# cbg-ethz/BnpC

Hardware: AMD Instinct MI355X
Metric: MCMC steps/s, 5k cells x 1k muts (+ cell x cluster log-lik evals/s in ll_evals_per_s_K0) (higher is better)
Workload: dtype f64

## Files before the change

### bnpc_amd/_lib.py

```python
import ctypes as C
import os
import re

import numpy as np

_PKG = os.path.dirname(os.path.abspath(__file__))
LIB_PATH = os.environ.get('BNPC_LIB') or os.path.join(_PKG, 'libbnpc_hip.so')

_environ_raw = getattr(os.environ, '_data', None)
if not isinstance(_environ_raw, dict) \
        or (_environ_raw and not isinstance(next(iter(_environ_raw)), bytes)):
    _environ_raw = None


def env(name, default=None):
    if _environ_raw is None:
        return os.environ.get(name, default)
    val = _environ_raw.get(name.encode() if isinstance(name, str) else name)
    return default if val is None else os.fsdecode(val)


MAX_VIEWS = 7
TILE_SLOTS = 4
MAX_TRIALS = 4
# ... 149 lines not shown
    'bnpc_view_set_slot': (C.c_int, [_ctx, C.c_int, _pi64, _i64, C.c_int]),
    'bnpc_view_size': (C.c_int, [_ctx, C.c_int, _pi64]),
    'bnpc_ll_theta': (C.c_int, [_ctx, C.c_int, _pf, _i64, C.c_double,
        C.c_double, _pd, _i64]),
    'bnpc_ll_theta_pinned': (C.c_int, [_ctx, C.c_int, _pf, _i64, C.c_double,
        C.c_double, _i64, _ppd]),
    'bnpc_ll_theta_pinned_top2': (C.c_int, [_ctx, C.c_int, _pf, _i64,
        C.c_double, C.c_double, _i64, _pd, _ppd, C.POINTER(C.c_void_p)]),
    'bnpc_ll_theta_pinned_top2_issue': (C.c_int, [_ctx, C.c_int, _pf, _i64,
        C.c_double, C.c_double, _i64, _pd, _ppd, C.POINTER(C.c_void_p)]),
    'bnpc_matrix_wait': (C.c_int, [_ctx]),
    'bnpc_hints_wait': (C.c_int, [_ctx]),
    'bnpc_ll_theta_pinned_sums_issue': (C.c_int, [_ctx, C.c_int, _pf, _i64,
        C.c_double, C.c_double, _i64, _pd, _ppd]),
    'bnpc_hints_in_order_issue': (C.c_int, [_ctx, _pi64,
        C.POINTER(C.c_void_p)]),
    'bnpc_theta_put': (C.c_int, [_ctx, _i64, _pf, _i64]),
    'bnpc_ll_rows_pinned': (C.c_int, [_ctx, C.c_int, _pi64, _i64, C.c_double,
        C.c_double, _i64, _ppd]),
    'bnpc_ll_rows_issue': (C.c_int, [_ctx, C.c_int, _pi64, _i64, C.c_double,
        C.c_double, _i64, C.c_int]),
    'bnpc_ll_rows_wait': (C.c_int, [_ctx, C.c_int, _ppd]),
    'bnpc_ll_rows_issue_hint': (C.c_int, [_ctx, C.c_int, _pi64, _i64,
        C.c_double, C.c_double, _i64, C.c_int, _pd]),
    'bnpc_ll_rows_wait_hint': (C.c_int, [_ctx, C.c_int, _ppd,
        C.POINTER(C.c_void_p)]),
    'bnpc_ll_tables': (C.c_int, [_ctx, C.c_int, _pd, _pd, _i64, _pd, _i64]),
    'bnpc_colcounts': (C.c_int, [_ctx, _pi64, _pi64, _i64, _pi32, _pi32]),
    'bnpc_view_counts': (C.c_int, [_ctx, C.c_int, _pi64, _i64, _pi32, _pi32]),
    'bnpc_colcounts_by_label': (C.c_int, [_ctx, _pi64, _pi64, _i64, _pi32,
# ... 71 lines not shown
        C.POINTER(C.c_void_p), C.POINTER(_i64)]),
    'bnpc_post_fetch': (C.c_int, [C.c_void_p, _pi32, _pd]),
    'bnpc_post_mpear': (C.c_int, [C.c_void_p, C.c_void_p, _i64, _pi64]),
    'bnpc_post_genotypes': (C.c_int, [C.c_void_p, _pi32, _i64, _pf, _i64,
        _i64, _i64, _pd]),
    'bnpc_post_ward': (C.c_int, [C.c_void_p, _pd]),
    'bnpc_post_ward_stats': (C.c_int, [C.c_void_p, C.POINTER(_i64),
        C.POINTER(_i64)]),
    'bnpc_post_destroy': (C.c_int, [C.c_void_p]),
    'bnpc_rg_scan': (C.c_int, [C.POINTER(MT19937), C.c_int, _i64, _pd,
        C.c_double, _pi64, _pi64, _pd]),
    'bnpc_mt_gamma': (C.c_int, [C.POINTER(MT19937), C.c_void_p, C.c_double,
        C.c_double, C.POINTER(C.c_double)]),
    'bnpc_chain_open': (C.c_int, [C.POINTER(ChainState)]),
    'bnpc_chain_close': (C.c_int, [C.POINTER(ChainState)]),
    'bnpc_chain_step': (C.c_int, [_ctx, C.c_void_p, C.POINTER(MT19937),
        C.POINTER(ChainState)]),
    'bnpc_chain_update_alpha': (C.c_int, [C.c_void_p, C.POINTER(MT19937),
        C.POINTER(ChainState)]),
    'bnpc_gamma_logpdf_scalar': (C.c_int, [C.c_void_p, C.c_double, C.c_double,
        C.c_double, C.POINTER(C.c_double), C.POINTER(C.c_int)]),
}

_lib = None


def load():
    global _lib
    if _lib is not None:
        return _lib
# ... 857 lines not shown
    return None if status.value else out.value


class NativeChain:

    def __init__(self, N, M):
        self.st = ChainState()
        self.st.N, self.st.M = N, M
        self.ids = np.zeros(N, dtype=np.int64)
        self.sizes = np.zeros(N, dtype=np.int64)
        self.st.ids, self.st.sizes = ptr(self.ids), ptr(self.sizes)
        self.keep = []
        self._lib = load()
        check(self._lib.bnpc_chain_open(C.byref(self.st)), 'chain_open')

    def close(self):
        if getattr(self, 'st', None) is not None and self.st.work:
            self._lib.bnpc_chain_close(C.byref(self.st))

    def __del__(self):
        try:
            self.close()
        except Exception:
            pass


def tn_ppf_scalar(kernels, q, a, b, loc, scale):
    out, status = C.c_double(0.0), C.c_int(0)
    check(load().bnpc_tn_ppf_scalar(C.addressof(kernels), q, a, b, loc, scale,
        C.byref(out), C.byref(status)), 'tn_ppf_scalar')
# ... 184 lines not shown
        check(self._lib.bnpc_hints_in_order_issue(self._h,
            ptr(order, C.c_int64), C.byref(hint)), 'hints_in_order_issue')
        if not hint.value or n == 0:
            return None
        raw = (C.c_char * (n * TOP2.itemsize)).from_address(hint.value)
        return np.frombuffer(raw, dtype=TOP2, count=n)

    def ll_theta_pinned_top2_in_order(self, view, theta, FP, FN, ld,
                col_prior, order):
        mat = self.ll_theta_pinned_sums_issue(view, theta, FP, FN, ld,
            col_prior)
        hint = self.hints_in_order_issue(order)
        self.hints_wait()
        return mat, hint

    def hints_wait(self):
        check(self._lib.bnpc_hints_wait(self._h), 'hints_wait')

    def matrix_wait(self):
        check(self._lib.bnpc_matrix_wait(self._h), 'matrix_wait')

    def matrix_wait_hook(self):
        return (C.cast(self._lib.bnpc_matrix_wait, C.c_void_p).value,
            self._h.value if hasattr(self._h, 'value') else self._h)

    def theta_put(self, row0, theta):
        theta = np.ascontiguousarray(theta, dtype=np.float32)
        if theta.ndim == 1:
            theta = theta[None, :]
        assert theta.shape[1] == self.M
# ... 198 lines not shown
```

### bnpc_amd/csrc/bnpc_ctx.h

```cpp
#ifndef BNPC_CTX_H
#define BNPC_CTX_H
#include <hip/hip_runtime.h>
#include <stdint.h>
#include <string.h>
#include <algorithm>
#include <vector>

#include "bnpc_hip.h"
#include "bnpc_internal.h"

#define HIPCHK(expr)                                                         \
    do {                                                                     \
        hipError_t e_ = (expr);                                              \
        if (e_ != hipSuccess) {                                              \
            bnpc_set_error("%s failed: %s (%s:%d)", #expr,                   \
                           hipGetErrorString(e_), __FILE__, __LINE__);       \
            return 1;                                                        \
        }                                                                    \
    } while (0)

#define ARGCHK(cond, msg)                                                    \
    do {                                                                     \
        if (!(cond)) {                                                       \
            bnpc_set_error("bad argument: %s", msg);                         \
// ... 85 lines not shown
    char *zc_out_dev = nullptr;
    void *hint_pin = nullptr;
    size_t hint_cap = 0;
    DevBuf hint_prior;
    void *hint_prior_pin = nullptr;
    struct {
        int state = 0;
        int64_t n = 0, K = 0, ldo = 0;
        size_t bytes = 0;
        Top2Prior prior;
        void *hint_dev = nullptr;
        double *rows_dev = nullptr;
    } hint_later;
    void *order_pin = nullptr;
    DevBuf order_dev;
    void *mh_pin = nullptr;
    char *mh_dev = nullptr;
    size_t mh_cap = 0;
    size_t mh_capE = 0;
    struct MhAhead *ahead = nullptr;
    int64_t ahead_begun = 0, ahead_taken = 0, ahead_rows_taken = 0;
    double mh_flagged_share = 0.25;
    hipEvent_t mh_ev[2] = {};
    int64_t screened = 0, screen_kept = 0;
    size_t pin_lazy_bytes = 0;
    bool matrix_eager = false, lazy_fetched = false, pin_copy_queued = false;
    hipEvent_t ev_hints = nullptr;
    unsigned *done_count = nullptr;
    unsigned *done_pin = nullptr;
    unsigned *done_dev = nullptr;
// ... 161 lines not shown
```

### bnpc_amd/csrc/bnpc_internal.h

```cpp
#ifndef BNPC_INTERNAL_H
#define BNPC_INTERNAL_H
#include <math.h>
#include <stdarg.h>
#include <stdint.h>

#include "bnpc_hip.h"

void bnpc_set_error(const char *fmt, ...);

#ifdef __cplusplus
#include <linux/futex.h>
#include <stdlib.h>
#include <sys/syscall.h>
#include <time.h>
#include <unistd.h>

#include <atomic>
#include <functional>
#include <thread>

static inline void bnpc_cpu_relax()
{
#if defined(__x86_64__)
    __builtin_ia32_pause();
// ... 69 lines not shown
                            int64_t *col_of_id, int64_t *col_id,
                            int64_t *col_size, int64_t *order);
double bnpc_legacy_gamma(bnpc_mt19937 *rng, bnpc_legacy_gauss *g, double shape,
                         double scale);

void bnpc_mh_rank0_hook(const std::function<void()> *hook);
void bnpc_mh_row_gate(const std::function<bool(int64_t)> *gate);
#ifdef __cplusplus
int bnpc_mh_ahead_begin(bnpc_ctx *c, const bnpc_mt19937 *rng,
                        const bnpc_legacy_gauss *g,
                        const std::function<bool(bnpc_mt19937 *,
                                                 bnpc_legacy_gauss *)> &prelude,
                        int64_t rows, int64_t M, int64_t n_sd, bool *posted,
                        int64_t min_entries = -1);
void bnpc_mh_ahead_drop(bnpc_ctx *c);
void bnpc_mh_ahead_scan(bnpc_ctx *c, const bnpc_mt19937 *rng, int64_t uniforms,
                        int64_t rows, int64_t M, int64_t n_sd);
void bnpc_rg_scan_order_hook(const std::function<void()> *hook);
void bnpc_move_last_draw_hook(const std::function<void(int)> *hook);
#endif
int bnpc_ll_theta_begin(bnpc_ctx *c, int view, const float *theta, int64_t K,
                        double FP, double FN, double *out, int64_t ldo);
int bnpc_ll_theta_end(bnpc_ctx *c);
int bnpc_rg_scan_step_with(bnpc_ctx *ctx, const bnpc_host_kernels *k,
                           bnpc_mt19937 *rng, int view, int64_t n,
                           int64_t *rg_assignment, double DP_a,
                           const bnpc_mh_args *mh, int32_t *n1, int32_t *n0,
                           double *scan_log_prob, int *status,
                           const double *ll_ready);
int bnpc_rg_counts_and_batch(bnpc_ctx *c, const bnpc_host_kernels *k,
// ... 141 lines not shown
```

### bnpc_amd/csrc/bnpc_kernels.hip

```cpp

#include <hip/hip_runtime.h>
#include <hip/hip_ext.h>
#include <stdint.h>
#include <stdio.h>
#include <stdlib.h>
#include <string.h>
#include <math.h>
#include <vector>
#include <algorithm>

#include "bnpc_ctx.h"

struct LaunchTimers {
    bool on = false;
    std::vector<hipEvent_t> ev;
    size_t used = 0;
    hipEvent_t *next_pair()
    {
        if (used + 2 > ev.size()) {
            const size_t old = ev.size();
            ev.resize(old + 512, nullptr);
            for (size_t i = old; i < ev.size(); i++)
                if (hipEventCreate(&ev[i]) != hipSuccess) {
                    ev.resize(i & ~(size_t)1);
// ... 677 lines not shown
    const double2 *__restrict__ src, double2 *__restrict__ dst, long long n2)
{
    const long long i = (long long)blockIdx.x * 256 + threadIdx.x;
    if (i < n2) dst[i] = src[i];
}

__device__ __forceinline__ void top2_floats(bnpc_top2 &t, double third,
    double fourth, double lb, double ls, double lt, bool has2, bool has3)
{
    t.third = __double2float_ru(third);
    t.fourth = __double2float_ru(fourth);
    t.e2 = has2 ? (float)exp(ls - lb) : 0.0f;
    t.e3 = has3 ? (float)exp(lt - lb) : 0.0f;
}

__global__ __launch_bounds__(256) void k_row_top2(
    const double *__restrict__ ll, long long n, long long ldo, int K,
    Top2Prior prior, bnpc_top2 *__restrict__ out,
    double *__restrict__ host_ll, const long long *__restrict__ order)
{
    const long long slot = (long long)blockIdx.x * 256 + threadIdx.x;
    if (slot >= n) return;
    const long long row = order ? order[slot] : slot;
    const double *__restrict__ r = ll + (size_t)row * ldo;
    double best = -INFINITY, second = -INFINITY, third = -INFINITY;
    double fourth = -INFINITY;
    double lb = 0.0, ls = 0.0, lt = 0.0;
    int col = 0, col2 = -1, col3 = -1;
    for (int k = 0; k < K; k++) {
        const double l = r[k];
        const double v = l + prior.v[k];
        if (v > best) {
            fourth = third;
            third = second;
            lt = ls;
            col3 = col2;
            second = best;
            ls = lb;
            col2 = best > -INFINITY ? col : -1;
            best = v;
            lb = l;
            col = k;
        } else if (v > second) {
            fourth = third;
            third = second;
            lt = ls;
            col3 = col2;
            second = v;
            ls = l;
            col2 = k;
        } else if (v > third) {
            fourth = third;
            third = v;
            lt = l;
            col3 = k;
        } else if (v > fourth) {
            fourth = v;
        }
    }
    bnpc_top2 t;
    t.best = best;
    t.second = second;
    t.ll_best = lb;
    t.ll_second = ls;
    t.ll_third = lt;
    t.col = (int16_t)col;
    t.col2 = (int16_t)col2;
    t.col3 = (int16_t)col3;
    top2_floats(t, third, fourth, lb, ls, lt, col2 >= 0, col3 >= 0);
    int through = 0;
    if (host_ll && (double)t.fourth > second - 72.0 && second > best - 48.0) {
        double *__restrict__ h = host_ll + (size_t)row * ldo;
        for (int k = 0; k < K; k++) h[k] = r[k];
        through = 1;
    }
    t.row_here = (int16_t)through;
    out[slot] = t;
}

struct Top4 {
    double b, s, t, f;
    double lb, ls, lt;
    int cb, cs, ct;
};

__device__ __forceinline__ bool top4_before(double v, int k, double x, int cx)
{
    return v > x || (v == x && k < cx);
}

__device__ __forceinline__ void top4_insert(Top4 &q, double v, double l, int k)
{
// ... 442 lines not shown
    }
    const int64_t cap = MSPLIT_MAX;
    if (tun.msplit_chunks > 0) want = (tun.msplit_chunks + 3) / 4 * 4;
    if (want > cap) want = cap;
    int chunk = (int)((Mt + want - 1) / want);
    chunk = (chunk + 7) / 8 * 8;
    if (chunk < 16) chunk = 16;
    const int ms = (Mt + chunk - 1) / chunk;
    if (ms >= 2) {
        *MS = ms;
        *m_chunk = chunk;
    }
}


template <int KW>
static int issue_ll(bnpc_ctx *c, const View &v, int64_t K, int64_t ldo,
                    double *d_out, int MS, int m_chunk)
{
    const int64_t G = (K + KW - 1) / KW;
    const int64_t nwg = ((v.nblk + 3) / 4) * G * MS;
    ARGCHK(nwg < (1ll << 31), "launch too large");
    const int xcd = 1;
    const size_t stream_bytes = (size_t)v.nblk * c->Mpad * 16
        + (size_t)G * c->Mt * 2 * KW * sizeof(double) / 8;
    const int pf = stream_bytes > (3u << 20) || MS > 1;
    double *dst = d_out;
    const int need_planes = MS > 1 ? (KW == 8 ? (MS + 3) / 4 : MS) : 1;
    if (need_planes > 1) {
        if (ensure(c->part, (size_t)need_planes * v.n * K * sizeof(double)))
// ... 51 lines not shown
            LAUNCH_ASM(1, false, nwg);
            snprintf(c->last_name, sizeof(c->last_name),
                     "k_ll8_asm<1, false>");
        }
    }
#undef LAUNCH_ASM
    else {
        snprintf(c->last_name, sizeof(c->last_name), "k_ll<%d>%s", KW,
                 MS > 1 ? " + k_ll_combine" : "");
        BNPC_LAUNCH(k_ll<KW>, dim3((unsigned)nwg), dim3(256), 0,
                           c->stream, (const ulonglong2 *)v.masks.p, c->Mpad,
                           c->Mt, (long long)v.n, (long long)v.nblk,
                           (const double *)c->tabs.p, (int)K, (long long)ldo,
                           dst, xcd, MS, m_chunk);
    }
    if (MS > 1 && planes > 1) {
        HIPCHK(hipGetLastError());
        const long long total = (long long)v.n * K;
        BNPC_LAUNCH(k_ll_combine, dim3((unsigned)((total + 255) / 256)),
                           dim3(256), 0, c->stream, (const double *)c->part.p,
                           (long long)v.n, (int)K, planes, (long long)ldo,
                           d_out, sig);
        c->sig_attached = sig.count != nullptr;
    } else if (KW == 8 && MS > 1 && need_planes == 1) {
        c->sig_attached = sig.count != nullptr;
    }
    HIPCHK(hipGetLastError());
    return 0;
}

template <int KW>
// ... 275 lines not shown
        HIPCHK(hipEventCreateWithFlags(&c->ev_hints, hipEventDisableTiming));
    HIPCHK(hipEventRecord(c->ev_hints, c->stream));
    if (c->matrix_eager) {
        HIPCHK(hipMemcpyAsync(c->pin, c->out.p, bytes, hipMemcpyDeviceToHost,
                              c->stream));
        c->pin_copy_queued = true;
    }
    if (wait) HIPCHK(hipEventSynchronize(c->ev_hints));
    c->pin_lazy_bytes = bytes;
    return 0;
}

static int ll_top2_impl(bnpc_ctx *c, int view, const float *theta, int64_t K,
                        double FP, double FN, int64_t ldo,
                        const double *col_prior, double **host,
                        bnpc_top2 **top2, bool wait, bool later = false)
{
    ARGCHK(c && host && col_prior && (top2 || later), "NULL argument");
    ARGCHK(K > 0 && K <= HINT_COLS_MAX, "K out of range for the hint");
    ARGCHK(view >= 0 && view < BNPC_MAX_VIEWS, "view out of range");
    if (top2) *top2 = nullptr;
    c->hint_later.state = 0;
    if (ldo == 0) ldo = K;
    const int64_t n = c->views[view].n;
    void *zc_dev = nullptr;
    bnpc_top2 *hint = nullptr;
    if (n && c->tun.zero_copy) {
        const size_t need = (size_t)n * sizeof(bnpc_top2);
        if (need > c->hint_cap) {
            if (c->hint_pin) HIPCHK(hipHostFree(c->hint_pin));
            c->hint_pin = nullptr;
// ... 30 lines not shown
            if (ensure(c->hint_prior, pb2)) return 1;
            if (!c->hint_prior_pin)
                HIPCHK(hipHostMalloc(&c->hint_prior_pin,
                                     ((size_t)HINT_COLS_MAX + 1) * 8,
                                     hipHostMallocDefault));
            void *pp_dev = nullptr;
            HIPCHK(hipHostGetDevicePointer(&pp_dev, c->hint_prior_pin, 0));
            memcpy(c->hint_prior_pin, col_prior, pb);
            const long long n2 = (long long)(pb2 / 16);
            BNPC_LAUNCH(k_stage_copy, dim3((unsigned)((n2 + 255) / 256)),
                               dim3(256), 0, c->stream, (const double2 *)pp_dev,
                               (double2 *)c->hint_prior.p, n2);
            HIPCHK(hipGetLastError());
        }
    }
    int rc = ll_theta_impl(c, view, theta, K, FP, FN, nullptr, ldo, false);
    if (rc) return rc;
    if (bytes == 0) {
        HIPCHK(hipStreamSynchronize(c->stream));
        if (later) c->hint_later.state = 2;
        return 0;
    }
    *host = (double *)c->pin;
    if (hint && later) {
        c->hint_later.state = 1;
        c->hint_later.n = n;
        c->hint_later.K = K;
        c->hint_later.ldo = ldo;
        c->hint_later.bytes = bytes;
        c->hint_later.prior = pr;
        c->hint_later.hint_dev = zc_dev;
// ... 52 lines not shown
    HIPCHK(hipStreamSynchronize(c->stream));
    return 0;
}

extern "C" int bnpc_ll_theta_pinned_sums_issue(bnpc_ctx *c, int view,
                                               const float *theta, int64_t K,
                                               double FP, double FN,
                                               int64_t ldo,
                                               const double *col_prior,
                                               double **host)
{
    return ll_top2_impl(c, view, theta, K, FP, FN, ldo, col_prior, host,
                        nullptr, false, true);
}

extern "C" int bnpc_hints_in_order_issue(bnpc_ctx *c, const int64_t *order,
                                         bnpc_top2 **top2)
{
    ARGCHK(c && order && top2, "NULL argument");
    *top2 = nullptr;
    HIPCHK(hipSetDevice(c->device));
    const int state = c->hint_later.state;
    c->hint_later.state = 0;
    ARGCHK(state != 0, "no sums issued for these hints "
                       "(bnpc_ll_theta_pinned_sums_issue comes first)");
    if (state == 2) return 0;
    const int64_t n = c->hint_later.n;
    ARGCHK(n <= c->N, "more rows than cells");
    {
        uint64_t out_of_range = 0;
        for (int64_t i = 0; i < n; i++)
            out_of_range |= (uint64_t)((uint64_t)order[i] >= (uint64_t)n);
        ARGCHK(!out_of_range, "order entry out of range");
    }
    const size_t ob = (size_t)n * sizeof(long long);
    const size_t ob2 = (ob + 15) & ~(size_t)15;
    if (!c->order_pin
        && hipHostMalloc(&c->order_pin, ((size_t)c->N + 2) * 8,
                         hipHostMallocDefault) != hipSuccess) {
        (void)hipGetLastError();
        c->order_pin = nullptr;
    }
    void *op_dev = nullptr;
    if (c->order_pin
// ... 1 lines not shown
        (void)hipGetLastError();
        op_dev = nullptr;
    }
    if (ensure(c->order_dev, ob2)) return 1;
    if (op_dev) {
        memcpy(c->order_pin, order, ob);
        const long long n2 = (long long)(ob2 / 16);
        BNPC_LAUNCH(k_stage_copy, dim3((unsigned)((n2 + 255) / 256)),
                    dim3(256), 0, c->stream, (const double2 *)op_dev,
                    (double2 *)c->order_dev.p, n2);
        HIPCHK(hipGetLastError());
    } else {
        HIPCHK(hipMemcpyAsync(c->order_dev.p, order, ob,
                              hipMemcpyHostToDevice, c->stream));
    }
    if (int rh = hint_launch(c, (const double *)c->out.p, n, c->hint_later.K,
                             c->hint_later.ldo, c->hint_later.prior,
                             c->hint_later.hint_dev, c->hint_later.rows_dev,
                             (const long long *)c->order_dev.p))
        return rh;
    if (int rq = hints_queued(c, c->hint_later.K, c->hint_later.bytes, false))
        return rq;
    *top2 = (bnpc_top2 *)c->hint_pin;
    return 0;
}

extern "C" int bnpc_hints_wait(bnpc_ctx *c)
{
    ARGCHK(c, "ctx is NULL");
    HIPCHK(hipSetDevice(c->device));
    if (c->ev_hints && c->pin_lazy_bytes)
        HIPCHK(hipEventSynchronize(c->ev_hints));
    else
        HIPCHK(hipStreamSynchronize(c->stream));
    return 0;
}

// ... 741 lines not shown
```

### bnpc_amd/csrc/bnpc_mhbatch.cpp

```cpp

#include <hip/hip_runtime.h>
#include <atomic>
#include <stdint.h>
#include <stdio.h>
#include <stdlib.h>
#include <string.h>
#include <time.h>
#include <functional>
#include <vector>
#include <algorithm>

#include "bnpc_ctx.h"

static size_t mh_pin_offsets(size_t E, size_t off[6])
{
    const size_t Ea = (E + 15) & ~(size_t)15;
    off[0] = 0;
    off[1] = off[0] + Ea * 8;
    off[2] = off[1] + Ea * 8;
    off[3] = off[2] + Ea * 4;
    off[4] = off[3] + Ea * 4;
    off[5] = off[4] + Ea * 4;
    return off[5] + Ea;
}
// ... 182 lines not shown
                break;
            ah->after_row[(size_t)r] = ah->rng;
            ah->rows_ready.store(r + 1, std::memory_order_release);
        }
    });
    if (!ok) return 0;
    ah->active = true;
    c->ahead_begun++;
    if (posted) *posted = true;
    return 0;
}

void bnpc_mh_ahead_drop(bnpc_ctx *c)
{
    if (c) mh_ahead_drop(c);
}

void bnpc_mh_ahead_scan(bnpc_ctx *c, const bnpc_mt19937 *rng, int64_t uniforms,
                        int64_t rows, int64_t M, int64_t n_sd)
{
    static const bnpc_legacy_gauss no_gauss = {};
    const auto way = [uniforms](bnpc_mt19937 *r, bnpc_legacy_gauss *) {
        for (int64_t left = 2 * uniforms; left > 0;) {
            if (r->pos >= 624) mt_refill(r);
            const int64_t take = std::min<int64_t>(624 - r->pos, left);
            r->pos += (int32_t)take;
            left -= take;
        }
        return true;
    };
// ... 488 lines not shown
```

### bnpc_amd/csrc/bnpc_step.cpp

```cpp
#include <stdio.h>
#include <stdlib.h>
#include <chrono>
#include <cstring>
#include <vector>

#include "bnpc_internal.h"

namespace {

const double EPSILON = 1e-15;

struct Memo {
    double key = 0.0, val = 0.0;
    bool set = false;
};

struct Work {
    int64_t N = 0, M = 0;
    std::vector<double> newcl, post_new;
    double newcl_FP = 0.0, newcl_FN = 0.0;
    bool newcl_set = false;
    std::vector<int64_t> perm, assign, col_of_id, col_id, col_size, order, born;
    std::vector<double> scratch, col_prior, heap_ll, tabs;
    std::vector<float> rows, fresh;
    bool rows_current = false;
    std::vector<int32_t> n1, n0;
    std::vector<int64_t> lab_ids, lab_assign;
    uint64_t lab_gen = 0;
    bool lab_set = false;
    std::vector<int64_t> pc_ids;
    std::vector<float> pc_theta, kt;
    std::vector<double> pc_prior, kp, prior_out, dens;
    bool pc_set = false;
// ... 194 lines not shown
            const int64_t take = std::min<int64_t>(624 - r->pos, left);
            r->pos += (int32_t)take;
            left -= take;
        }
        if (mt_double(r) < dpa_prob) {
            double alpha;
            if (alpha_draws(k, r, g, args, &alpha)) return false;
        }
        return true;
    };
    bool posted = false;
    (void)bnpc_mh_ahead_begin(ctx, rng, (const bnpc_legacy_gauss *)ch->gauss,
                              way, ch->K + 1, ch->M, ch->n_sd, &posted);
}

int gibbs_phase(bnpc_ctx *ctx, const bnpc_host_kernels *k, bnpc_mt19937 *rng,
                bnpc_chain *ch, Work &w, bool *done)
{
    *done = false;
    const Clock::time_point tg_in = Clock::now();
    const int64_t N = ch->N, M = ch->M, K = ch->K;
    const int64_t spare = K <= 64
        ? std::max<int64_t>(4, std::min<int64_t>(16, K / 4))
        : std::min<int64_t>(512, std::max<int64_t>(16, K / 8));
    if (K < 1 || K + 512 > 32767 || !ch->sweep_hint || ch->param_stride != M
        || ch->sweep_bytes / (8 * (K + spare)) < N)
        return 0;
    const double FP = ch->FP, FN = ch->FN;
    if (!w.newcl_set || w.newcl_FP != FP || w.newcl_FN != FN) {
        const double c1 = np_log1(k, ch->mix1 * (1 - FN) + ch->mix0 * FP);
// ... 21 lines not shown
        if (ch->sizes[g] < 1 || ch->sizes[g] > N) {
            bnpc_set_error("bad argument: cluster size out of range");
            return 2;
        }
        w.col_prior[g] = ch->crp_prior[ch->sizes[g]];
    }
    static const bool trace_g = [] {
        const char *e = getenv("BNPC_TIMING");
        return e && strstr(e, "gibbs");
    }();
    const Clock::time_point tg0 = Clock::now();
    gather_rows(ch, w);
    const Clock::time_point tg1 = Clock::now();
    double *ll = nullptr;
    bnpc_top2 *top2 = nullptr;
    int rc = bnpc_ll_theta_pinned_sums_issue(ctx, 0, w.rows.data(), K, FP, FN,
                                             ld, w.col_prior.data(), &ll);
    if (rc) return rc;
    const Clock::time_point tg2 = Clock::now();
    w.perm.resize((size_t)N);
    mt_fill_permutation(rng, N, w.perm.data());
    rc = bnpc_hints_in_order_issue(ctx, w.perm.data(), &top2);
    if (rc) return rc;
    if (ch->phase == BNPC_PHASE_ASSIGN) params_ahead(ctx, k, rng, ch, N);
    w.assign.assign(ch->assignment, ch->assignment + N);
    w.col_of_id.assign((size_t)N, -1);
    w.col_id.assign((size_t)ld, -1);
    w.col_size.assign((size_t)ld, 0);
    w.order.assign((size_t)ld, 0);
    for (int64_t g = 0; g < K; g++) {
        const int64_t id = ch->ids[g];
        if (id < 0 || id >= N || w.col_of_id[id] >= 0) {
            (void)bnpc_hints_wait(ctx);
            bnpc_set_error("bad argument: cluster ids");
            return 2;
        }
        w.col_of_id[id] = g;
        w.col_id[g] = id;
// ... 98 lines not shown
    memcpy(ch->assignment, w.assign.data(), (size_t)N * 8);
    ch->swept += N;
    ch->hint_used += st.hint_used;
    ch->pair_used += st.pair_used;
    ch->triple_used += st.triple_used;
    ch->lane_used += st.lane_used;
    ch->stride_used += st.stride_used;
    std::vector<double>().swap(w.heap_ll);
    if (trace_g) {
        auto us = [](Clock::time_point a, Clock::time_point b) {
            return std::chrono::duration_cast<std::chrono::nanoseconds>(
                b - a).count() / 1e3;
        };
        fprintf(stderr, "[gibbs] N=%lld K=%lld: new-cluster term + priors "
                "%.1f, rows %.1f, issue %.1f, order + hints issue + state "
                "%.1f, wait %.1f, loop %.1f, commit %.1f us\n", (long long)N,
                (long long)K, us(tg_in, tg0), us(tg0, tg1), us(tg1, tg2),
                us(tg2, tg3), us(tg3, tg4), us(tg4, tg5),
                us(tg5, Clock::now()));
    }
    *done = true;
    return 0;
}

int move_phase(bnpc_ctx *ctx, const bnpc_host_kernels *k, bnpc_mt19937 *rng,
               bnpc_chain *ch, Work &w, int move, bool *done)
{
    *done = false;
    if (!k->gammaln) return 0;
    bnpc_move_state st;
    memset(&st, 0, sizeof st);
    st.move = move;
    st.scan_no = ch->sm_steps;
// ... 368 lines not shown
{
    if (!ch || ch->N < 1 || ch->M < 1) {
        bnpc_set_error("bad argument: chain_open");
        return 2;
    }
    Work *w = new Work();
    w->N = ch->N;
    w->M = ch->M;
    ch->work = w;
    return 0;
}

extern "C" int bnpc_chain_close(bnpc_chain *ch)
{
    if (ch && ch->work) {
        delete (Work *)ch->work;
        ch->work = nullptr;
    }
    return 0;
}

extern "C" int bnpc_chain_step(bnpc_ctx *ctx, const bnpc_host_kernels *k,
                               bnpc_mt19937 *rng, bnpc_chain *ch)
{
    if (!ctx || !k || !rng || !ch || !ch->work || !ch->assignment
        || !ch->parameters || !ch->ids || !ch->sizes || !ch->crp_prior
        || !ch->sd || !ch->gauss || ch->n_sd < 1 || ch->K < 1
        || ch->K > ch->N || ch->param_stride < ch->M
        || ch->phase < BNPC_PHASE_ASSIGN || ch->phase > BNPC_PHASE_RECORD) {
        bnpc_set_error("bad argument: chain_step");
        return 2;
    }
    Work &w = *(Work *)ch->work;
// ... 84 lines not shown
            Lap lap(ch, 5);
            rc = alpha_phase(k, rng, ch, w);
            if (rc) return rc;
            lap.stop();
        }
    }
    if (ch->phase <= BNPC_PHASE_PARAMS) {
        Lap lap(ch, 6);
        rc = params_phase(ctx, k, rng, ch, w, &done);
        if (rc) return rc;
        if (!done) {
            ch->need = BNPC_NEED_PARAMS;
            return 0;
        }
        lap.stop();
    }
    if (ch->phase <= BNPC_PHASE_ERRORS && ch->learning) {
        if (mt_double(rng) < ch->error_prob) {
            Lap lap(ch, 7);
            const Snapshot before(rng, gauss);
            const double FP0 = ch->FP, FN0 = ch->FN;
            rc = ensure_counts(ctx, ch, w);
            if (rc) return rc;
            gather_rows(ch, w);
            for (int which = 0; which < 2; which++) {
                rc = error_rate(ctx, k, rng, ch, w, which, &done);
                if (rc) return rc;
                if (!done) {
                    before.put_back(rng, gauss);
                    ch->FP = FP0;
// ... 26 lines not shown
```

### bnpc_amd/model.py

```python
import ctypes as C
import os

import numpy as np
from scipy.special import gamma as _gamma_fn, gammaln
from scipy.stats import beta as _beta_dist, truncnorm
from scipy.stats import gamma as _gamma_dist

from bnpc_amd import _lib, fastdist, hostkernels

np.seterr(divide='raise', over='ignore', under='ignore', invalid='raise')

EPSILON = np.finfo(np.float64).resolution
TMIN = 1e-5
TMAX = 1 - TMIN
log_EPSILON = np.log(EPSILON)

_THREAD_MIN_ELEMS = 1 << 14
_ELEMS_PER_THREAD = 8192
_POOL = {}


def _host_parts(elems, rows):
    if elems < _THREAD_MIN_ELEMS or rows < 2:
        return 1
# ... 1112 lines not shown
            'pair_used': getattr(self, '_pair_used', 0),
            'triple_used': getattr(self, '_triple_used', 0),
            'lane_used': getattr(self, '_lane_used', 0),
            'stride_used': getattr(self, '_stride_used', 0),
            'native_moves': getattr(self, '_native_moves', 0),
            'native_steps': getattr(self, '_native_steps', 0)}
        nat = getattr(self, '_nat', None)
        if nat is not None:
            for key in ('swept', 'hint_used', 'pair_used', 'triple_used',
                    'lane_used', 'stride_used', 'native_moves'):
                out[key] += getattr(nat.st, key)
        ctx = getattr(self, '_ctx', None)
        ahead = getattr(ctx, 'mh_ahead_stats', None)
        out['ahead_begun'], out['ahead_taken'], out['ahead_rows'] = \
            ahead() if ahead is not None else (0, 0, 0)
        return out

    def update_parameters(self, step_no=None):
        ids = np.fromiter(self.cells_per_cluster.keys(), dtype=np.int64)
        lab = self._lab
        stale = lab is None or not np.array_equal(lab['ids'], ids) \
            or not np.array_equal(lab['assignment'], self.assignment)
        ctx = self._dev()
        table = _native_kernels()
        if stale and table is not None and getattr(ctx, '_h', None):
            old = self.parameters[ids]
            n1 = np.empty(old.shape, dtype=np.int32)
            n0 = np.empty(old.shape, dtype=np.int32)
            status, new, _, declined, prior, draws = _lib.mh_batch(
                table, old, n1, n0, self.param_proposal_sd, TMIN, TMAX,
# ... 692 lines not shown
```

### include/bnpc_hip.h

```cpp
#ifndef BNPC_HIP_H
#define BNPC_HIP_H

#include <stdint.h>

#ifdef __cplusplus
extern "C" {
#endif

typedef struct bnpc_ctx bnpc_ctx;

#define BNPC_MAX_VIEWS 7
#define BNPC_TILE_SLOTS 4
#define BNPC_MAX_TRIALS 4

const char *bnpc_last_error(void);
int bnpc_abi_version(void);
int bnpc_device_count(int *count);
int bnpc_device_info(int device, char *name, int len, int *cus);

int bnpc_device_pci_bus_id(int device, char *bus_id, int len);

int bnpc_team_stress(int64_t jobs, int max_tasks, int ranks, uint64_t seed,
                     int64_t *done, int64_t *expected);
int bnpc_team_size(int threads);
// ... 43 lines not shown
                              int64_t K, double FP, double FN, int64_t ldo,
                              const double *col_prior, double **host,
                              bnpc_top2 **top2);
int bnpc_ll_theta_pinned_top2_issue(bnpc_ctx *ctx, int view,
                                    const float *theta, int64_t K, double FP,
                                    double FN, int64_t ldo,
                                    const double *col_prior, double **host,
                                    bnpc_top2 **top2);
int bnpc_hints_wait(bnpc_ctx *ctx);
int bnpc_ll_theta_pinned_sums_issue(bnpc_ctx *ctx, int view,
                                    const float *theta, int64_t K, double FP,
                                    double FN, int64_t ldo,
                                    const double *col_prior, double **host);
int bnpc_hints_in_order_issue(bnpc_ctx *ctx, const int64_t *order,
                              bnpc_top2 **top2);
int bnpc_matrix_wait(bnpc_ctx *ctx);

int bnpc_theta_put(bnpc_ctx *ctx, int64_t row0, const float *theta, int64_t R);
int bnpc_ll_rows_pinned(bnpc_ctx *ctx, int view, const int64_t *rows,
                        int64_t K, double FP, double FN, int64_t ldo,
                        double **host);

int bnpc_ll_rows_issue(bnpc_ctx *ctx, int view, const int64_t *rows, int64_t K,
                       double FP, double FN, int64_t ldo, int slot);
int bnpc_ll_rows_wait(bnpc_ctx *ctx, int slot, double **host);
int bnpc_ll_rows_issue_hint(bnpc_ctx *ctx, int view, const int64_t *rows,
                            int64_t K, double FP, double FN, int64_t ldo,
                            int slot, const double *col_prior);
int bnpc_ll_rows_wait_hint(bnpc_ctx *ctx, int slot, double **host,
                           bnpc_top2 **hint);
// ... 280 lines not shown
    int32_t alpha_updated, errors_updated, FP_accepted, FN_accepted;
    int64_t par_declined, par_accepted;
    int32_t rec_params_done, pad_;
    double ML, lprior;
    int64_t swept, hint_used, pair_used, triple_used, native_moves, steps;
    int64_t lane_used;
    int64_t stride_used;
    int64_t clock_ns[BNPC_STEP_CLOCKS], clock_calls[BNPC_STEP_CLOCKS];
    void *work;
} bnpc_chain;

int bnpc_chain_open(bnpc_chain *ch);
int bnpc_chain_close(bnpc_chain *ch);
int bnpc_chain_step(bnpc_ctx *ctx, const bnpc_host_kernels *k,
                    bnpc_mt19937 *rng, bnpc_chain *ch);
int bnpc_chain_update_alpha(const bnpc_host_kernels *k, bnpc_mt19937 *rng,
                            bnpc_chain *ch);
int bnpc_gamma_logpdf_scalar(const bnpc_host_kernels *k, double x, double a,
                             double loc, double *out, int *status);

int bnpc_parse_matrix(const char *path, char sep, int skip_rows,
                      int skip_index, int8_t *out, int64_t *rows,
                      int64_t *cols);
int bnpc_write_table(const char *path, int64_t R, int64_t K, const char *blob,
                     const int64_t *off, int64_t N, const int32_t *col);

int bnpc_codist(int device, const int32_t *assignments, int64_t S, int64_t N,
                int32_t *differ);

typedef struct bnpc_post bnpc_post;
// ... 18 lines not shown
```

Baseline: 2931.

## Precompute Gibbs sweep permutation ahead and fuse partial-sum combine with top2 hints

After: 2775. 0.947x the previous value.

```diff
diff --git a/bnpc_amd/_lib.py b/bnpc_amd/_lib.py
--- a/bnpc_amd/_lib.py
+++ b/bnpc_amd/_lib.py
@@ -187,6 +187,9 @@
     'bnpc_ll_theta_pinned_sums_issue': (C.c_int, [_ctx, C.c_int, _pf, _i64,
         C.c_double, C.c_double, _i64, _pd, _ppd]),
     'bnpc_hints_in_order_issue': (C.c_int, [_ctx, _pi64,
+        C.POINTER(C.c_void_p)]),
+    'bnpc_ll_theta_pinned_sums_hints_issue': (C.c_int, [_ctx, C.c_int, _pf,
+        _i64, C.c_double, C.c_double, _i64, _pd, _pi64, _ppd,
         C.POINTER(C.c_void_p)]),
     'bnpc_theta_put': (C.c_int, [_ctx, _i64, _pf, _i64]),
     'bnpc_ll_rows_pinned': (C.c_int, [_ctx, C.c_int, _pi64, _i64, C.c_double,
@@ -288,6 +291,10 @@
         C.c_double, C.POINTER(C.c_double)]),
     'bnpc_chain_open': (C.c_int, [C.POINTER(ChainState)]),
     'bnpc_chain_close': (C.c_int, [C.POINTER(ChainState)]),
+    'bnpc_chain_order_ahead_stats': (C.c_int, [C.POINTER(ChainState),
+        C.POINTER(C.c_int64), C.POINTER(C.c_int64)]),
+    'bnpc_chain_order_ahead_hook': (C.c_int, [C.POINTER(ChainState),
+        C.POINTER(MT19937), C.c_int, C.c_int, _pi64, C.POINTER(C.c_int)]),
     'bnpc_chain_step': (C.c_int, [_ctx, C.c_void_p, C.POINTER(MT19937),
         C.POINTER(ChainState)]),
     'bnpc_chain_update_alpha': (C.c_int, [C.c_void_p, C.POINTER(MT19937),
@@ -1175,6 +1182,12 @@
         self._lib = load()
         check(self._lib.bnpc_chain_open(C.byref(self.st)), 'chain_open')
 
+    def order_ahead_stats(self):
+        b, t = C.c_int64(), C.c_int64()
+        check(self._lib.bnpc_chain_order_ahead_stats(C.byref(self.st),
+            C.byref(b), C.byref(t)), 'chain_order_ahead_stats')
+        return b.value, t.value
+
     def close(self):
         if getattr(self, 'st', None) is not None and self.st.work:
             self._lib.bnpc_chain_close(C.byref(self.st))
@@ -1389,6 +1402,27 @@
         self.hints_wait()
         return mat, hint
 
+    def ll_theta_pinned_sums_hints_issue(self, view, theta, FP, FN, ld,
+                col_prior, order):
+        theta = np.ascontiguousarray(theta, dtype=np.float32)
+        K = theta.shape[0]
+        col_prior = np.ascontiguousarray(col_prior, dtype=np.float64)
+        order = as_i64(order)
+        n = self.view_size(view)
+        assert col_prior.size == K and order.size == n
+        host, hint = _host_pd(), C.c_void_p()
+        check(self._lib.bnpc_ll_theta_pinned_sums_hints_issue(self._h, view,
+            ptr(theta, C.c_float), K, float(FP), float(FN), ld,
+            ptr(col_prior), ptr(order, C.c_int64), C.byref(host),
+            C.byref(hint)), 'll_theta_pinned_sums_hints_issue')
+        if n == 0:
+            return np.empty((0, ld)), None
+        mat = np.ctypeslib.as_array(host, shape=(n, ld))
+        if not hint.value:
+            return mat, None
+        raw = (C.c_char * (n * TOP2.itemsize)).from_address(hint.value)
+        return mat, np.frombuffer(raw, dtype=TOP2, count=n)
+
     def hints_wait(self):
         check(self._lib.bnpc_hints_wait(self._h), 'hints_wait')
 
diff --git a/bnpc_amd/csrc/bnpc_ctx.h b/bnpc_amd/csrc/bnpc_ctx.h
--- a/bnpc_amd/csrc/bnpc_ctx.h
+++ b/bnpc_amd/csrc/bnpc_ctx.h
@@ -123,6 +123,14 @@
     } hint_later;
     void *order_pin = nullptr;
     DevBuf order_dev;
+    struct {
+        bool want = false, done = false;
+        Top2Prior prior;
+        bnpc_top2 *hint_dev = nullptr;
+        double *rows_dev = nullptr;
+        const int64_t *order = nullptr;
+    } fuse;
+    std::vector<uint8_t> order_seen;
     void *mh_pin = nullptr;
     char *mh_dev = nullptr;
     size_t mh_cap = 0;
diff --git a/bnpc_amd/csrc/bnpc_internal.h b/bnpc_amd/csrc/bnpc_internal.h
--- a/bnpc_amd/csrc/bnpc_internal.h
+++ b/bnpc_amd/csrc/bnpc_internal.h
@@ -107,6 +107,7 @@
                         int64_t rows, int64_t M, int64_t n_sd, bool *posted,
                         int64_t min_entries = -1);
 void bnpc_mh_ahead_drop(bnpc_ctx *c);
+int bnpc_ctx_mh_ahead_mode(const bnpc_ctx *c);
 void bnpc_mh_ahead_scan(bnpc_ctx *c, const bnpc_mt19937 *rng, int64_t uniforms,
                         int64_t rows, int64_t M, int64_t n_sd);
 void bnpc_rg_scan_order_hook(const std::function<void()> *hook);
diff --git a/bnpc_amd/csrc/bnpc_kernels.hip b/bnpc_amd/csrc/bnpc_kernels.hip
--- a/bnpc_amd/csrc/bnpc_kernels.hip
+++ b/bnpc_amd/csrc/bnpc_kernels.hip
@@ -715,22 +715,14 @@
     t.e3 = has3 ? (float)exp(lt - lb) : 0.0f;
 }
 
-__global__ __launch_bounds__(256) void k_row_top2(
-    const double *__restrict__ ll, long long n, long long ldo, int K,
-    Top2Prior prior, bnpc_top2 *__restrict__ out,
-    double *__restrict__ host_ll, const long long *__restrict__ order)
-{
-    const long long slot = (long long)blockIdx.x * 256 + threadIdx.x;
-    if (slot >= n) return;
-    const long long row = order ? order[slot] : slot;
-    const double *__restrict__ r = ll + (size_t)row * ldo;
+struct RowTop {
     double best = -INFINITY, second = -INFINITY, third = -INFINITY;
     double fourth = -INFINITY;
     double lb = 0.0, ls = 0.0, lt = 0.0;
     int col = 0, col2 = -1, col3 = -1;
-    for (int k = 0; k < K; k++) {
-        const double l = r[k];
-        const double v = l + prior.v[k];
+
+    __device__ __forceinline__ void put(double l, double v, int k)
+    {
         if (v > best) {
             fourth = third;
             third = second;
@@ -759,24 +751,99 @@
             fourth = v;
         }
     }
+
+    __device__ __forceinline__ bool record(bnpc_top2 &t) const
+    {
+        t.best = best;
+        t.second = second;
+        t.ll_best = lb;
+        t.ll_second = ls;
+        t.ll_third = lt;
+        t.col = (int16_t)col;
+        t.col2 = (int16_t)col2;
+        t.col3 = (int16_t)col3;
+        top2_floats(t, third, fourth, lb, ls, lt, col2 >= 0, col3 >= 0);
+        return (double)t.fourth > second - 72.0 && second > best - 48.0;
+    }
+};
+
+__global__ __launch_bounds__(256) void k_row_top2(
+    const double *__restrict__ ll, long long n, long long ldo, int K,
+    Top2Prior prior, bnpc_top2 *__restrict__ out,
+    double *__restrict__ host_ll, const long long *__restrict__ order)
+{
+    const long long slot = (long long)blockIdx.x * 256 + threadIdx.x;
+    if (slot >= n) return;
+    const long long row = order ? order[slot] : slot;
+    const double *__restrict__ r = ll + (size_t)row * ldo;
+    RowTop top;
+    for (int k = 0; k < K; k++) {
+        const double l = r[k];
+        top.put(l, l + prior.v[k], k);
+    }
     bnpc_top2 t;
-    t.best = best;
-    t.second = second;
-    t.ll_best = lb;
-    t.ll_second = ls;
-    t.ll_third = lt;
-    t.col = (int16_t)col;
-    t.col2 = (int16_t)col2;
-    t.col3 = (int16_t)col3;
-    top2_floats(t, third, fourth, lb, ls, lt, col2 >= 0, col3 >= 0);
+    const bool scan = top.record(t);
     int through = 0;
-    if (host_ll && (double)t.fourth > second - 72.0 && second > best - 48.0) {
+    if (host_ll && scan) {
         double *__restrict__ h = host_ll + (size_t)row * ldo;
         for (int k = 0; k < K; k++) h[k] = r[k];
         through = 1;
     }
     t.row_here = (int16_t)through;
     out[slot] = t;
+}
+
+__global__ __launch_bounds__(256) void k_ll_combine_top2(
+    const double *__restrict__ part, long long n, int K, int MS,
+    long long ldo, double *__restrict__ out, Top2Prior prior,
+    bnpc_top2 *__restrict__ hint, double *__restrict__ host_ll,
+    const long long *__restrict__ order, DoneSignal done)
+{
+    const int j = threadIdx.x & 15;
+    const int lane0 = (threadIdx.x & 63) & ~15;
+    const long long slot = (long long)blockIdx.x * 16 + (threadIdx.x >> 4);
+    const bool valid = slot < n;
+    const long long row = valid ? order[slot] : 0;
+    const size_t stride = (size_t)n * K;
+    const double *__restrict__ p = part + (size_t)row * K + j;
+    double s[4];
+#pragma unroll
+    for (int c = 0; c < 4; c++) s[c] = j + 16 * c < K ? p[16 * c] : 0.0;
+#pragma unroll 4
+    for (int ms = 1; ms < MS; ms++) {
+        const double *__restrict__ q = p + (size_t)ms * stride;
+#pragma unroll
+        for (int c = 0; c < 4; c++)
+            if (j + 16 * c < K) s[c] += q[16 * c];
+    }
+    if (valid) {
+        double *__restrict__ o = out + (size_t)row * ldo + j;
+#pragma unroll
+        for (int c = 0; c < 4; c++)
+            if (j + 16 * c < K) o[16 * c] = s[c];
+    }
+    RowTop top;
+#pragma unroll
+    for (int c = 0; c < 4; c++)
+        for (int i = 0; i < 16 && 16 * c + i < K; i++) {
+            const double l = __shfl(s[c], lane0 + i);
+            top.put(l, l + prior.v[16 * c + i], 16 * c + i);
+        }
+    bnpc_top2 t;
+    const bool scan = top.record(t);
+    int through = 0;
+    if (host_ll && scan) {
+        if (valid) {
+            double *__restrict__ h = host_ll + (size_t)row * ldo + j;
+#pragma unroll
+            for (int c = 0; c < 4; c++)
+                if (j + 16 * c < K) h[16 * c] = s[c];
+        }
+        through = 1;
+    }
+    t.row_here = (int16_t)through;
+    if (valid && j == 0) hint[slot] = t;
+    signal_done(done);
 }
 
 struct Top4 {
@@ -1249,6 +1316,9 @@
 }
 
 
+static int order_stage(bnpc_ctx *c, const int64_t *order, int64_t n,
+                       bool permutation);
+
 template <int KW>
 static int issue_ll(bnpc_ctx *c, const View &v, int64_t K, int64_t ldo,
                     double *d_out, int MS, int m_chunk)
@@ -1330,7 +1400,20 @@
                            (const double *)c->tabs.p, (int)K, (long long)ldo,
                            dst, xcd, MS, m_chunk);
     }
-    if (MS > 1 && planes > 1) {
+    if (MS > 1 && planes > 1 && c->fuse.want && K <= 64) {
+        HIPCHK(hipGetLastError());
+        if (int ro = order_stage(c, c->fuse.order, v.n, true)) return ro;
+        BNPC_LAUNCH(k_ll_combine_top2, dim3((unsigned)((v.n + 15) / 16)),
+                           dim3(256), 0, c->stream, (const double *)c->part.p,
+                           (long long)v.n, (int)K, planes, (long long)ldo,
+                           d_out, c->fuse.prior, c->fuse.hint_dev,
+                           c->fuse.rows_dev,
+                           (const long long *)c->order_dev.p, sig);
+        c->sig_attached = sig.count != nullptr;
+        c->fuse.done = true;
+        const size_t at = strlen(c->last_name);
+        snprintf(c->last_name + at, sizeof(c->last_name) - at, "_top2");
+    } else if (MS > 1 && planes > 1) {
         HIPCHK(hipGetLastError());
         const long long total = (long long)v.n * K;
         BNPC_LAUNCH(k_ll_combine, dim3((unsigned)((total + 255) / 256)),
@@ -1636,7 +1719,8 @@
 static int ll_top2_impl(bnpc_ctx *c, int view, const float *theta, int64_t K,
                         double FP, double FN, int64_t ldo,
                         const double *col_prior, double **host,
-                        bnpc_top2 **top2, bool wait, bool later = false)
+                        bnpc_top2 **top2, bool wait, bool later = false,
+                        const int64_t *fuse_order = nullptr)
 {
     ARGCHK(c && host && col_prior && (top2 || later), "NULL argument");
     ARGCHK(K > 0 && K <= HINT_COLS_MAX, "K out of range for the hint");
@@ -1697,7 +1781,16 @@
             HIPCHK(hipGetLastError());
         }
     }
+    c->fuse.done = false;
+    if (fuse_order && hint && bytes && K <= 64) {
+        c->fuse.prior = pr;
+        c->fuse.hint_dev = (bnpc_top2 *)zc_dev;
+        c->fuse.rows_dev = rows_dev;
+        c->fuse.order = fuse_order;
+        c->fuse.want = true;
+    }
     int rc = ll_theta_impl(c, view, theta, K, FP, FN, nullptr, ldo, false);
+    c->fuse.want = false;
     if (rc) return rc;
     if (bytes == 0) {
         HIPCHK(hipStreamSynchronize(c->stream));
@@ -1780,20 +1873,22 @@
                         nullptr, false, true);
 }
 
-extern "C" int bnpc_hints_in_order_issue(bnpc_ctx *c, const int64_t *order,
-                                         bnpc_top2 **top2)
-{
-    ARGCHK(c && order && top2, "NULL argument");
-    *top2 = nullptr;
-    HIPCHK(hipSetDevice(c->device));
-    const int state = c->hint_later.state;
-    c->hint_later.state = 0;
-    ARGCHK(state != 0, "no sums issued for these hints "
-                       "(bnpc_ll_theta_pinned_sums_issue comes first)");
-    if (state == 2) return 0;
-    const int64_t n = c->hint_later.n;
+static int order_stage(bnpc_ctx *c, const int64_t *order, int64_t n,
+                       bool permutation)
+{
     ARGCHK(n <= c->N, "more rows than cells");
-    {
+    if (permutation) {
+        c->order_seen.assign((size_t)n, 0);
+        uint64_t bad = 0;
+        for (int64_t i = 0; i < n; i++) {
+            const uint64_t r = (uint64_t)order[i] < (uint64_t)n
+                ? (uint64_t)order[i] : 0;
+            bad |= (uint64_t)((uint64_t)order[i] >= (uint64_t)n)
+                | c->order_seen[(size_t)r];
+            c->order_seen[(size_t)r] = 1;
+        }
+        ARGCHK(!bad, "order is not a permutation of the rows");
+    } else {
         uint64_t out_of_range = 0;
         for (int64_t i = 0; i < n; i++)
             out_of_range |= (uint64_t)((uint64_t)order[i] >= (uint64_t)n);
@@ -1825,13 +1920,59 @@
         HIPCHK(hipMemcpyAsync(c->order_dev.p, order, ob,
                               hipMemcpyHostToDevice, c->stream));
     }
-    if (int rh = hint_launch(c, (const double *)c->out.p, n, c->hint_later.K,
-                             c->hint_later.ldo, c->hint_later.prior,
-                             c->hint_later.hint_dev, c->hint_later.rows_dev,
+    return 0;
+}
+
+static int hints_later_launch(bnpc_ctx *c, bnpc_top2 **top2)
+{
+    if (int rh = hint_launch(c, (const double *)c->out.p, c->hint_later.n,
+                             c->hint_later.K, c->hint_later.ldo,
+                             c->hint_later.prior, c->hint_later.hint_dev,
+                             c->hint_later.rows_dev,
                              (const long long *)c->order_dev.p))
         return rh;
     if (int rq = hints_queued(c, c->hint_later.K, c->hint_later.bytes, false))
         return rq;
+    *top2 = (bnpc_top2 *)c->hint_pin;
+    return 0;
+}
+
+extern "C" int bnpc_hints_in_order_issue(bnpc_ctx *c, const int64_t *order,
+                                         bnpc_top2 **top2)
+{
+    ARGCHK(c && order && top2, "NULL argument");
+    *top2 = nullptr;
+    HIPCHK(hipSetDevice(c->device));
+    const int state = c->hint_later.state;
+    c->hint_later.state = 0;
+    ARGCHK(state != 0, "no sums issued for these hints "
+                       "(bnpc_ll_theta_pinned_sums_issue comes first)");
+    if (state == 2) return 0;
+    if (int rc = order_stage(c, order, c->hint_later.n, false)) return rc;
+    return hints_later_launch(c, top2);
+}
+
+extern "C" int bnpc_ll_theta_pinned_sums_hints_issue(
+    bnpc_ctx *c, int view, const float *theta, int64_t K, double FP,
+    double FN, int64_t ldo, const double *col_prior, const int64_t *order,
+    double **host, bnpc_top2 **top2)
+{
+    ARGCHK(c && order && top2, "NULL argument");
+    ARGCHK(view >= 0 && view < BNPC_MAX_VIEWS, "view out of range");
+    *top2 = nullptr;
+    HIPCHK(hipSetDevice(c->device));
+    const int64_t n = c->views[view].n;
+    if (int rc = ll_top2_impl(c, view, theta, K, FP, FN, ldo, col_prior, host,
+                              nullptr, false, true, order))
+        return rc;
+    const int state = c->hint_later.state;
+    c->hint_later.state = 0;
+    if (state != 1) return 0;
+    if (!c->fuse.done) {
+        if (int rc = order_stage(c, order, n, true)) return rc;
+        return hints_later_launch(c, top2);
+    }
+    if (int rq = hints_queued(c, K, c->hint_later.bytes, false)) return rq;
     *top2 = (bnpc_top2 *)c->hint_pin;
     return 0;
 }
diff --git a/bnpc_amd/csrc/bnpc_mhbatch.cpp b/bnpc_amd/csrc/bnpc_mhbatch.cpp
--- a/bnpc_amd/csrc/bnpc_mhbatch.cpp
+++ b/bnpc_amd/csrc/bnpc_mhbatch.cpp
@@ -220,6 +220,11 @@
 void bnpc_mh_ahead_drop(bnpc_ctx *c)
 {
     if (c) mh_ahead_drop(c);
+}
+
+int bnpc_ctx_mh_ahead_mode(const bnpc_ctx *c)
+{
+    return c ? c->tun.mh_ahead : 0;
 }
 
 void bnpc_mh_ahead_scan(bnpc_ctx *c, const bnpc_mt19937 *rng, int64_t uniforms,
diff --git a/bnpc_amd/csrc/bnpc_step.cpp b/bnpc_amd/csrc/bnpc_step.cpp
--- a/bnpc_amd/csrc/bnpc_step.cpp
+++ b/bnpc_amd/csrc/bnpc_step.cpp
@@ -1,5 +1,6 @@
 #include <stdio.h>
 #include <stdlib.h>
+#include <atomic>
 #include <chrono>
 #include <cstring>
 #include <vector>
@@ -15,8 +16,21 @@
     bool set = false;
 };
 
+struct OrderAhead {
+    bnpc_mt19937 rng;
+    double error_prob = 0.0, sm_prob = 0.0;
+    bool learning = false;
+    int64_t N = 0;
+    bool active = false;
+    std::atomic<int> known{0};
+    bnpc_mt19937 start, after;
+    std::vector<int64_t> perm;
+};
+
 struct Work {
     int64_t N = 0, M = 0;
+    OrderAhead order_ahead;
+    int64_t order_begun = 0, order_adopted = 0;
     std::vector<double> newcl, post_new;
     double newcl_FP = 0.0, newcl_FN = 0.0;
     bool newcl_set = false;
@@ -241,6 +255,71 @@
                               way, ch->K + 1, ch->M, ch->n_sd, &posted);
 }
 
+void order_ahead_wait(Work &w)
+{
+    OrderAhead &oa = w.order_ahead;
+    if (!oa.active) return;
+    while (oa.known.load(std::memory_order_acquire) == 0) bnpc_aside_wait();
+    oa.active = false;
+}
+
+void order_ahead_post(int mode, const bnpc_mt19937 *rng, const bnpc_chain *ch,
+                      Work &w)
+{
+    order_ahead_wait(w);
+    if (ch->fix_assign || !ch->sweep_hint || ch->param_stride != ch->M
+        || mode == 0)
+        return;
+    OrderAhead *oa = &w.order_ahead;
+    oa->rng = *rng;
+    oa->error_prob = ch->error_prob;
+    oa->sm_prob = ch->sm_prob;
+    oa->learning = ch->learning != 0;
+    oa->N = ch->N;
+    oa->known.store(0, std::memory_order_relaxed);
+    const bool ok = bnpc_aside_start([oa]() {
+        bnpc_mt19937 *r = &oa->rng;
+        if (oa->learning && mt_double(r) < oa->error_prob)
+            for (int which = 0; which < 2; which++) {
+                (void)mt_interval(r, 2);
+                (void)mt_double(r);
+                (void)mt_double(r);
+            }
+        if (mt_double(r) < oa->sm_prob) {
+            oa->known.store(-1, std::memory_order_release);
+            return;
+        }
+        if (r->pos >= 624) mt_refill(r);
+        oa->start = *r;
+        oa->perm.resize((size_t)oa->N);
+        mt_fill_permutation(r, oa->N, oa->perm.data());
+        oa->after = *r;
+        oa->known.store(1, std::memory_order_release);
+    });
+    if (!ok) return;
+    oa->active = true;
+    w.order_begun++;
+}
+
+bool order_ahead_take(int mode, bnpc_mt19937 *rng, Work &w, int64_t N)
+{
+    OrderAhead &oa = w.order_ahead;
+    if (!oa.active) return false;
+    order_ahead_wait(w);
+    if (oa.known.load(std::memory_order_acquire) != 1 || oa.N != N
+        || mode == 3)
+        return false;
+    bnpc_mt19937 live = *rng;
+    if (live.pos >= 624) mt_refill(&live);
+    if (live.pos != oa.start.pos
+        || memcmp(live.key, oa.start.key, sizeof live.key) != 0)
+        return false;
+    w.perm.swap(oa.perm);
+    *rng = oa.after;
+    w.order_adopted++;
+    return true;
+}
+
 int gibbs_phase(bnpc_ctx *ctx, const bnpc_host_kernels *k, bnpc_mt19937 *rng,
                 bnpc_chain *ch, Work &w, bool *done)
 {
@@ -292,14 +371,29 @@
     const Clock::time_point tg1 = Clock::now();
     double *ll = nullptr;
     bnpc_top2 *top2 = nullptr;
-    int rc = bnpc_ll_theta_pinned_sums_issue(ctx, 0, w.rows.data(), K, FP, FN,
+    int rc;
+    Clock::time_point tg2, tg2a, tg2b;
+    const bool ahead = order_ahead_take(bnpc_ctx_mh_ahead_mode(ctx), rng, w,
+                                        N);
+    if (ahead) {
+        rc = bnpc_ll_theta_pinned_sums_hints_issue(ctx, 0, w.rows.data(), K,
+                                                   FP, FN, ld,
+                                                   w.col_prior.data(),
+                                                   w.perm.data(), &ll, &top2);
+        if (rc) return rc;
+        tg2 = tg2a = tg2b = Clock::now();
+    } else {
+        rc = bnpc_ll_theta_pinned_sums_issue(ctx, 0, w.rows.data(), K, FP, FN,
                                              ld, w.col_prior.data(), &ll);
-    if (rc) return rc;
-    const Clock::time_point tg2 = Clock::now();
-    w.perm.resize((size_t)N);
-    mt_fill_permutation(rng, N, w.perm.data());
-    rc = bnpc_hints_in_order_issue(ctx, w.perm.data(), &top2);
-    if (rc) return rc;
+        if (rc) return rc;
+        tg2 = Clock::now();
+        w.perm.resize((size_t)N);
+        mt_fill_permutation(rng, N, w.perm.data());
+        tg2a = Clock::now();
+        rc = bnpc_hints_in_order_issue(ctx, w.perm.data(), &top2);
+        if (rc) return rc;
+        tg2b = Clock::now();
+    }
     if (ch->phase == BNPC_PHASE_ASSIGN) params_ahead(ctx, k, rng, ch, N);
     w.assign.assign(ch->assignment, ch->assignment + N);
     w.col_of_id.assign((size_t)N, -1);
@@ -428,9 +522,11 @@
         };
         fprintf(stderr, "[gibbs] N=%lld K=%lld: new-cluster term + priors "
                 "%.1f, rows %.1f, issue %.1f, order + hints issue + state "
-                "%.1f, wait %.1f, loop %.1f, commit %.1f us\n", (long long)N,
+                "%.1f (order %s %.1f, hints issue %.1f, state %.1f), wait "
+                "%.1f, loop %.1f, commit %.1f us\n", (long long)N,
                 (long long)K, us(tg_in, tg0), us(tg0, tg1), us(tg1, tg2),
-                us(tg2, tg3), us(tg3, tg4), us(tg4, tg5),
+                us(tg2, tg3), ahead ? "ahead" : "drawn", us(tg2, tg2a),
+                us(tg2a, tg2b), us(tg2b, tg3), us(tg3, tg4), us(tg4, tg5),
                 us(tg5, Clock::now()));
     }
     *done = true;
@@ -829,9 +925,41 @@
 extern "C" int bnpc_chain_close(bnpc_chain *ch)
 {
     if (ch && ch->work) {
+        order_ahead_wait(*(Work *)ch->work);
         delete (Work *)ch->work;
         ch->work = nullptr;
     }
+    return 0;
+}
+
+extern "C" int bnpc_chain_order_ahead_hook(bnpc_chain *ch, bnpc_mt19937 *rng,
+                                           int mode, int take, int64_t *order,
+                                           int *adopted)
+{
+    if (!ch || !ch->work || !rng || (take && (!order || !adopted))) {
+        bnpc_set_error("bad argument: chain_order_ahead_hook");
+        return 2;
+    }
+    Work &w = *(Work *)ch->work;
+    if (!take) {
+        order_ahead_post(mode, rng, ch, w);
+        return 0;
+    }
+    *adopted = order_ahead_take(mode, rng, w, ch->N) ? 1 : 0;
+    if (*adopted) memcpy(order, w.perm.data(), (size_t)ch->N * 8);
+    return 0;
+}
+
+extern "C" int bnpc_chain_order_ahead_stats(const bnpc_chain *ch,
+                                            int64_t *begun, int64_t *adopted)
+{
+    if (!ch || !ch->work || !begun || !adopted) {
+        bnpc_set_error("bad argument: chain_order_ahead_stats");
+        return 2;
+    }
+    const Work &w = *(const Work *)ch->work;
+    *begun = w.order_begun;
+    *adopted = w.order_adopted;
     return 0;
 }
 
@@ -946,6 +1074,7 @@
             return 0;
         }
         lap.stop();
+        order_ahead_post(bnpc_ctx_mh_ahead_mode(ctx), rng, ch, w);
     }
     if (ch->phase <= BNPC_PHASE_ERRORS && ch->learning) {
         if (mt_double(rng) < ch->error_prob) {
diff --git a/bnpc_amd/model.py b/bnpc_amd/model.py
--- a/bnpc_amd/model.py
+++ b/bnpc_amd/model.py
@@ -1150,6 +1150,8 @@
         ahead = getattr(ctx, 'mh_ahead_stats', None)
         out['ahead_begun'], out['ahead_taken'], out['ahead_rows'] = \
             ahead() if ahead is not None else (0, 0, 0)
+        out['order_begun'], out['order_adopted'] = \
+            nat.order_ahead_stats() if nat is not None else (0, 0)
         return out
 
     def update_parameters(self, step_no=None):
diff --git a/include/bnpc_hip.h b/include/bnpc_hip.h
--- a/include/bnpc_hip.h
+++ b/include/bnpc_hip.h
@@ -81,6 +81,12 @@
                                     const double *col_prior, double **host);
 int bnpc_hints_in_order_issue(bnpc_ctx *ctx, const int64_t *order,
                               bnpc_top2 **top2);
+int bnpc_ll_theta_pinned_sums_hints_issue(bnpc_ctx *ctx, int view,
+                                          const float *theta, int64_t K,
+                                          double FP, double FN, int64_t ldo,
+                                          const double *col_prior,
+                                          const int64_t *order, double **host,
+                                          bnpc_top2 **top2);
 int bnpc_matrix_wait(bnpc_ctx *ctx);
 
 int bnpc_theta_put(bnpc_ctx *ctx, int64_t row0, const float *theta, int64_t R);
@@ -391,6 +397,10 @@
 int bnpc_chain_close(bnpc_chain *ch);
 int bnpc_chain_step(bnpc_ctx *ctx, const bnpc_host_kernels *k,
                     bnpc_mt19937 *rng, bnpc_chain *ch);
+int bnpc_chain_order_ahead_stats(const bnpc_chain *ch, int64_t *begun,
+                                 int64_t *adopted);
+int bnpc_chain_order_ahead_hook(bnpc_chain *ch, bnpc_mt19937 *rng, int mode,
+                                int take, int64_t *order, int *adopted);
 int bnpc_chain_update_alpha(const bnpc_host_kernels *k, bnpc_mt19937 *rng,
                             bnpc_chain *ch);
 int bnpc_gamma_logpdf_scalar(const bnpc_host_kernels *k, double x, double a,
```
